# JanWosnitza/FrayTracer

Hardware: AMD Instinct MI355X
Metric: Mrays/s (primary+secondary) at 4096x4096; max per-pixel |delta| vs F# ref (delta is measured against the CPU oracle: F# parity is unpinned, DESIGN.md section 2) (higher is better)
Workload: dtype f32

## Files before the change

fraytracer_amd/csrc/kernels.hip:

```cpp
#include <hip/hip_runtime.h>

#include "../../include/fraytracer_hip.h"
#include "ft_device.h"
#include "ft_kernels.h"
#include "ft_math.h"
#include "ft_libm.h"

#define FT_CONST __attribute__((address_space(4)))
typedef const float FT_CONST* cfp;
template <class T> __device__ __forceinline__ const T FT_CONST* as_const(const T* p) {
    return (const T FT_CONST*)(p);
}

__device__ __forceinline__ f3 ld3(cfp c) { return mk3(c[0], c[1], c[2]); }
__device__ __forceinline__ FtInstr ld_instr(const FtInstr FT_CONST* q) {
    FtInstr r; r.op = q->op; r.dst = q->dst; r.src = q->src; r.type = q->type; r.count = q->count; r.data = q->data;
    r.aux = q->aux; r.flags = q->flags; r.f0 = q->f0; r.f1 = q->f1; r.pad0 = 0; r.pad1 = 0; return r;
}
typedef float v4f __attribute__((ext_vector_type(4)));
typedef uint32_t v4u __attribute__((ext_vector_type(4)));
struct ItemRegs { v4f a; v4u b; };
__device__ __forceinline__ ItemRegs ld_item(const FtItemRec FT_CONST* q) {
    ItemRegs r;
    r.a = *reinterpret_cast<const v4f FT_CONST*>(q);
// ... 990 lines not shown
    float* o = out + 3ull * idx;
    o[0] = c.x; o[1] = c.y; o[2] = c.z;
}

__device__ __forceinline__ f3 ft_background(const FtRenderArgs& a) { return mk3(a.S.bg[0], a.S.bg[1], a.S.bg[2]); }

__device__ __forceinline__ const FtRenderArgs& ft_args_reread() {
    const FtRenderArgs FT_CONST* p = (const FtRenderArgs FT_CONST*)__builtin_amdgcn_kernarg_segment_ptr();
    asm volatile("" : "+s"(p));
    return *(const FtRenderArgs*)p;
}
#define FT_ARGS_AT_USE(on, a) ((on) ? ft_args_reread() : (a))

template <bool EXT>
__device__ __forceinline__ void emit(const FtRenderArgs& a, const LaneState& s, f3 c) {
    write_rgb(a.out, s.outIdx, EXT ? c * s.thr : c);
}

__device__ __forceinline__ uint32_t ft_glass_hash(uint32_t seed, uint32_t bounce) {
    uint32_t h = seed + (bounce + 1u) * 0x27D4EB2Fu;
    h ^= h >> 16; h *= 0x7FEB352Du; h ^= h >> 15; h *= 0x846CA68Bu; h ^= h >> 16;
    return h;
}

__device__ __forceinline__ void write_try_trace_miss(const FtRenderArgs& a, const LaneState& s) {
    float* o = a.out + 10ull * s.outIdx;
    for (uint32_t i = 0; i < 10u; ++i) o[i] = 0.0f;
}
__device__ __forceinline__ void write_ray(float* o, f3 origin, f3 dir, float len, float eps) {
    o[0] = origin.x; o[1] = origin.y; o[2] = origin.z; o[3] = dir.x; o[4] = dir.y; o[5] = dir.z; o[6] = len; o[7] = eps;
}

template <bool VIEWS = false>
__device__ __forceinline__ bool ends_hit_segment(const FtRenderArgs& a, const LaneState& s) {
    if (VIEWS) return a.hits != 0u && (s.job / a.jobsPerPlane) % a.spp == 0u && s.bounce() == 0u;
    return a.hits != 0u && s.job < a.jobsPerPlane && s.bounce() == 0u;
}
template <bool VIEWS = false>
__device__ __forceinline__ uint32_t hit_index(const FtRenderArgs& a, const LaneState& s) {
    if (!VIEWS) return s.outIdx;
    const uint32_t plane = s.job / a.jobsPerPlane;
    return s.outIdx - (plane - plane / a.spp) * a.planePixels;
}
__device__ __forceinline__ void write_hit_record(const FtRenderArgs& a, uint32_t idx, v4f r0, v4f r1, v4f r2, v4f r3, int32_t handle) {
    if (a.hitsOut != nullptr) {
        v4f* o = reinterpret_cast<v4f*>(a.hitsOut + 16ull * idx);
        o[0] = r0; o[1] = r1; o[2] = r2; o[3] = r3;
    }
    if (a.matOut != nullptr) a.matOut[idx] = handle;
}
__device__ __forceinline__ void write_hit_miss(const FtRenderArgs& a, uint32_t idx) {
    const v4f z = {0.0f, 0.0f, 0.0f, 0.0f};
    write_hit_record(a, idx, z, z, z, z, -1);
}

__device__ __forceinline__ bool ft_never_enters(const FtSceneDev& S, const f3 o, const f3 dir, float eps, float len) {
    if (!(S.escR >= 0.0f) || !(len < 1e9f) || !(eps >= 0.0f) || !(eps <= S.escR)) return false;
    const f3 w = o - mk3(S.escC[0], S.escC[1], S.escC[2]);
    const float re = S.escR + eps;
    const float ww = ft_dot(w, w), cc = ww - re * re, tol = 4e-6f * ww, dd = ft_dot(dir, dir);
    if (!(cc > tol) || !(dd < 1e12f)) return false;
    const bool longRay = dd >= 0.25f && ww <= S.escRho2;
    const bool shortRay = len <= 9.9f * S.escR && 2.0f * (ww + dd * (len * len)) <= 6.2f * (S.escR * S.escR);
    if (!longRay && !shortRay) return false;
    const float b = ft_dot(w, dir);
    if (b >= 0.0f) return true;
    return cc * dd - b * b > tol * dd;
}

__device__ __forceinline__ bool ft_cert_segment(const FtSceneDev& S, bool test, const f3 o, const f3 dir, float eps, float len, uint32_t steps,
                                                float& t0, float& t1) {
    const f3 w = o - mk3(S.escC[0], S.escC[1], S.escC[2]);
    const float ww = ft_dot(w, w), dd = ft_dot(dir, dir), b = ft_dot(w, dir);
    bool ok = test && S.certM >= 0.0f && S.escR >= 0.0f && eps >= 0.0f && eps <= S.escR && len > 0.0f && len < 1e9f && dd >= 0.81f && dd <= 1.44f &&
              ww <= S.certRho2 && steps < FT_STEP_CAP - S.certSteps;
    const float R = (S.escR + eps + S.certClip) * 1.001f;
    const float disc = b * b - dd * (ww - R * R);
    ok = ok && disc > 0.0f;
    const float sq = __builtin_amdgcn_sqrtf(ok ? disc : 0.0f), idd = 1.0f / dd;
    t0 = __builtin_fmaxf((-b - sq) * idd, 0.0f); t1 = __builtin_fminf((sq - b) * idd, len * S.certLenF);
    return ok && t1 > t0;
}

template <class P>
__device__ __forceinline__ float ft_seg_dist2(const P prm, const f3 p0, const f3 sv, const float iss) {
    const float vx = prm.x - p0.x, vy = prm.y - p0.y, vz = prm.z - p0.z;
    float t = __builtin_fmaf(vz, sv.z, __builtin_fmaf(vy, sv.y, vx * sv.x)) * iss;
    t = __builtin_amdgcn_fmed3f(t, 0.0f, 1.0f);
    const float ex = __builtin_fmaf(-t, sv.x, vx), ey = __builtin_fmaf(-t, sv.y, vy), ez = __builtin_fmaf(-t, sv.z, vz);
    return __builtin_fmaf(ez, ez, __builtin_fmaf(ey, ey, ex * ex));
}

__device__ __forceinline__ float ft_cert_threshold(float xt) { return __builtin_amdgcn_exp2f(xt) * 0.9999f; }

__device__ __forceinline__ bool ft_miss_certificate(const FtSceneDev& S, const float* __restrict__ ldsC, bool test, const f3 o, const f3 dir, float eps, float len,
                                                    uint32_t steps) {
    const FtInstr FT_CONST* in = as_const(S.instr);
    const float si = in->f0;
    const uint32_t n = in->count;
    const float4* c = reinterpret_cast<const float4*>(ldsC + in->data);
    float t0, t1;
    bool ok = ft_cert_segment(S, test, o, dir, eps, len, steps, t0, t1);
    const float A = si * 1.44269504f;
    const float xt = A * (eps + S.certM);
    ok = ok && xt >= -100.0f;
    if (__ballot(ok) == 0ull) return false;
    const float thr = ft_cert_threshold(xt);
    const f3 p0 = ok ? o + dir * t0 : mk3(0.0f, 0.0f, 0.0f);
    const f3 sv = ok ? dir * (t1 - t0) : mk3(1.0f, 0.0f, 0.0f);
    const float iss = 1.0f / ft_dot(sv, sv);
    float sum = 0.0f;
    uint32_t i = 0;
    auto term = [&](const auto prm) { return __builtin_amdgcn_exp2f((__builtin_amdgcn_sqrtf(ft_seg_dist2(prm, p0, sv, iss)) - prm.w) * A); };
    if (S.certK != 0u) {
        const v4f FT_CONST* cl = reinterpret_cast<const v4f FT_CONST*>(as_const(S.certCl));
        const v4f FT_CONST* kid = cl + 2u * S.certK;
        const float mthr = thr * (0.5f / (float)S.certK);
        float all = 0.0f, rest = 0.0f;
        uint32_t mark = 0u;
        for (uint32_t k = 0; k < S.certK; ++k) {
            const float bnd = term(cl[2u * k]) * (float)__float_as_uint(cl[2u * k + 1u].x);
            all += bnd;
            if (bnd >= mthr) mark |= 1u << k;
            else rest += bnd;
        }
        const bool held = ok && all < thr, open = ok && !held;
        if (__ballot(open) == 0ull) return held;
        float exact = 0.0f;
        for (uint32_t k = 0; k < S.certK; ++k) {
            const bool mine = (mark >> k) & 1u;
            if (__ballot(open && mine) == 0ull) continue;
            const v4f r = cl[2u * k + 1u];
            const uint32_t cnt = __float_as_uint(r.x), first = __float_as_uint(r.y);
            float part = 0.0f;
            for (uint32_t j = 0; j < cnt; ++j) part += term(kid[first + j]);
            exact += mine ? part : 0.0f;
            if (__ballot(open && exact < thr) == 0ull) return held;
        }
        return held || (open && rest + exact < thr);
    }
    for (; i + 8u <= n; i += 8u) {
#pragma unroll
        for (int j = 0; j < 8; ++j) sum += term(c[i + j]);
        if (__ballot(ok && sum < thr) == 0ull) return false;
    }
    for (; i < n; ++i) sum += term(c[i]);
    return ok && sum < thr;
}

__device__ __forceinline__ int ft_axis_lane(unsigned long long mm) {
    return (mm >> 27) != 0ull ? 26 + __ffsll((long long)(mm >> 27)) : __ffsll((long long)mm) - 1;
}

template <bool LEAN = false>
__device__ __forceinline__ bool ft_bundle_certificate(const FtSceneDev& S, const float* __restrict__ ldsC, bool cand, const f3 o, const f3 dir, float eps, float len,
                                                      uint32_t steps, uint32_t minMembers) {
    float t0, t1;
    const bool mem = ft_cert_segment(S, cand, o, dir, eps, len, steps, t0, t1);
    const unsigned long long mm = __ballot(mem);
    if (mm == 0ull || (uint32_t)__popcll(mm) < minMembers) return false;
    const FtInstr FT_CONST* in = as_const(S.instr);
    const float A = in->f0 * 1.44269504f;
    const uint32_t n = in->count;
    const float4* c = reinterpret_cast<const float4*>(ldsC + in->data);
    const int ax = ft_axis_lane(mm);
    const f3 oc = ft_readlane3(o, ax), dc = ft_readlane3(dir, ax);
    const float tc0 = ft_readlane_f(t0, ax), tc1 = ft_readlane_f(t1, ax);
    const f3 g = o - oc, h = dir - dc;
    const float sl = ft_dot(g, dc) * (1.0f / ft_dot(dc, dc));
    const float ex = __builtin_fmaf(-sl, dc.x, g.x), ey = __builtin_fmaf(-sl, dc.y, g.y), ez = __builtin_fmaf(-sl, dc.z, g.z);
    const float al = __builtin_amdgcn_sqrtf(__builtin_fmaf(ez, ez, __builtin_fmaf(ey, ey, ex * ex)));
    const float bl = __builtin_amdgcn_sqrtf(__builtin_fmaf(h.z, h.z, __builtin_fmaf(h.y, h.y, h.x * h.x)));
    const float Wr = ft_wave_max<LEAN>(mem ? __builtin_fmaf(bl, t1, al) : 0.0f);
    const float epsMax = ft_wave_max<LEAN>(mem ? eps : 0.0f);
    const float Rc = (S.escR + epsMax + S.certClip) * 1.001f;
    const float W = Wr * 1.001f + (1e-6f + 4e-6f * Rc);
    const float xt = A * (epsMax + S.certM);
    if (!(W <= S.escR) || !(xt >= -100.0f)) return false;
    const float dLo = ft_wave_max<LEAN>(mem ? __builtin_fmaxf(tc1 - (sl + t0), 0.0f) : 0.0f);
    const float dHi = ft_wave_max<LEAN>(mem ? __builtin_fmaxf((sl + t1) - tc0, 0.0f) : 0.0f);
    const float i0 = (tc1 - dLo) - 4e-6f * Rc, i1 = (tc0 + dHi) + 4e-6f * Rc;
    const f3 p0 = oc + dc * i0, sv = dc * (i1 - i0);
    const float iss = 1.0f / ft_dot(sv, sv);
    const float thr = ft_cert_threshold(xt);
    const uint32_t lane = threadIdx.x & 63u;
    float sum = 0.0f;
    for (uint32_t base = 0; base < n; base += 64u) {
        const uint32_t i = base + lane;
        const float4 prm = c[i < n ? i : n - 1u];
        const float term = __builtin_amdgcn_exp2f((__builtin_amdgcn_sqrtf(ft_seg_dist2(prm, p0, sv, iss)) - (prm.w + W)) * A);
        sum += i < n ? term : 0.0f;
        if (LEAN && __ballot(sum >= thr) != 0ull) return false;
    }
    float total;
    ft_wave_scan_incl(sum, total);
    return mem && total < thr;
}

template <bool LEAN = false>
__device__ __forceinline__ bool ft_occlusion_certificate(const FtRenderArgs& a, const float* __restrict__ ldsC, bool cand, const f3 o, const f3 dir, float eps, float len,
                                                         uint32_t steps) {
    const FtSceneDev& S = a.S;
    const f3 w = o - mk3(S.escC[0], S.escC[1], S.escC[2]);
    const float dd = ft_dot(dir, dir);
    const bool ok = cand && a.occ.b >= 0.0f && S.escR >= 0.0f && eps >= a.occ.epsMin && eps <= S.escR && len > 0.0f && len < 1e9f && dd >= 0.81f && dd <= 1.000001f &&
                    ft_dot(w, w) <= S.certRho2 && steps < FT_STEP_CAP / 2u;
    const unsigned long long mm = __ballot(ok);
    if (mm == 0ull) return false;
    const FtInstr FT_CONST* in = as_const(S.instr);
    const uint32_t n = in->count;
    const float si = in->f0;
    const float4* c = reinterpret_cast<const float4*>(ldsC + in->data);
    const float tEnd = len * a.occ.lenInv;
    const int ax = ft_axis_lane(mm);
    const f3 oc = ft_readlane3(o, ax), dc = ft_readlane3(dir, ax);
    const float tc = ft_readlane_f(tEnd, ax), idc = 1.0f / ft_dot(dc, dc);
    const uint32_t lane = threadIdx.x & 63u;
    auto approach = [](const f3 p, const f3 q, const f3 e, const float ie, const float tMaxi, float& t) {
        const float vx = p.x - q.x, vy = p.y - q.y, vz = p.z - q.z;
        t = __builtin_amdgcn_fmed3f(__builtin_fmaf(vz, e.z, __builtin_fmaf(vy, e.y, vx * e.x)) * ie, 0.0f, tMaxi);
        const float ex = __builtin_fmaf(-t, e.x, vx), ey = __builtin_fmaf(-t, e.y, vy), ez = __builtin_fmaf(-t, e.z, vz);
        return __builtin_amdgcn_sqrtf(__builtin_fmaf(ez, ez, __builtin_fmaf(ey, ey, ex * ex)));
    };
    float best = 0.0f, tAx;
    uint32_t bi = 0u;
    for (uint32_t base = 0; base < n; base += 64u) {
        const uint32_t i = base + lane;
        const float4 prm = c[i < n ? i : n - 1u];
        const float nr = (prm.w + a.occ.near) - approach(mk3(prm.x, prm.y, prm.z), oc, dc, idc, tc, tAx);
        if (i < n && nr > best) { best = nr; bi = i; }
    }
    const float nearest = ft_wave_max<LEAN>(best);
    if (!(nearest > 0.0f)) return false;
    const int src = __ffsll((long long)__ballot(best == nearest)) - 1;
    const float4 sp = c[(uint32_t)__builtin_amdgcn_readlane((int)bi, src)];
    (void)approach(mk3(sp.x, sp.y, sp.z), oc, dc, idc, tc, tAx);
    const f3 y = oc + dc * tAx;
    const float A = si * 1.44269504f;
    float sum = 0.0f;
    for (uint32_t base = 0; base < n; base += 64u) {
        const uint32_t i = base + lane;
        const float4 prm = c[i < n ? i : n - 1u];
        const float dx = prm.x - y.x, dy = prm.y - y.y, dz = prm.z - y.z;
        const float term = __builtin_amdgcn_exp2f((__builtin_amdgcn_sqrtf(__builtin_fmaf(dz, dz, __builtin_fmaf(dy, dy, dx * dx))) - prm.w) * A);
        sum += i < n ? term : 0.0f;
    }
    float total;
    ft_wave_scan_incl(sum, total);
    const float D = __builtin_amdgcn_logf(total) * (-0.693147181f / si);
    const float ie = 1.0f / eps, idd = 1.0f / dd;
    float t;
    bool holds = false;
    {
        const float dist = approach(mk3(sp.x, sp.y, sp.z), o, dir, idd, tEnd, t);
        const float nSteps = __builtin_fmaf(t, ie, 2.0f), hitM = __builtin_fmaf(a.occ.e, nSteps, a.occ.b);
        holds = t <= a.occ.reach && nSteps < 131072.0f && hitM <= a.occ.cap && (dist + hitM) * 1.001f < sp.w;
    }
    {
        const float dist = approach(y, o, dir, idd, tEnd, t);
        const float nSteps = __builtin_fmaf(t, ie, 2.0f), hitM = __builtin_fmaf(a.occ.e, nSteps, a.occ.b);
        holds = holds || (t <= a.occ.reach && nSteps < 131072.0f && hitM <= a.occ.cap && (dist + hitM) * 1.001f < D);
    }
    return ok && holds;
}

__device__ __forceinline__ int first_step_from_cache(LaneState& s) {
    if (s.len <= 0.0f) return 0;
    const float d = *ft_sh(FT_SH_D0);
    if (d != d) { ft_flag(1u); return 2; }
    if (d < s.eps) return 1;
    s.o = s.o + s.dir * d;
    s.len = s.len - d;
    s.steps = 1;
    return 0;
}

struct FtLit { f3 lint, ldir; };
__device__ __forceinline__ FtLit ft_light_at(const uint32_t type, const f3 lv, const f3 lc, const f3 hp) {
    f3 lint = lc, ldir = lv;
    if (type != FT_LIGHT_DIRECTIONAL) { ldir = ft_normalize(lv - hp); lint = lint / ft_length2(lv - hp); }
    return FtLit{lint, ldir};
}

template <bool EXT, int FORM = FT_FORM_FRAME, bool LEAN = false>
__device__ __forceinline__ void settle(const FtRenderArgs& a, LaneState& s) {
    constexpr bool VIEWS = FORM == FT_FORM_VIEWS, SHADE = FORM == FT_FORM_SHADE || FORM == FT_FORM_VIS, VIS = FORM == FT_FORM_VIS;
    const float piInv = 1.0f / 3.14159274101257324f;
    const FtRenderArgs* u = &a;
    for (;;) {
        if (!SHADE && s.phase == PH_MARCH) {
            if (s.len <= 0.0f || ((!EXT || !s.inside()) && ft_never_enters(a.S, s.o, s.dir, s.eps, s.len))) {
                if (LEAN) u = &ft_args_reread();
                if (EXT && u->mode == 2u) write_try_trace_miss(*u, s);
                else {
                    if (EXT && ends_hit_segment<VIEWS>(*u, s)) write_hit_miss(*u, hit_index<VIEWS>(*u, s));
                    if (!EXT || u->hits != 2u) emit<EXT>(*u, s, ft_background(*u));
                }
                s.phase = PH_IDLE;
            }
            return;
        }
        if (EXT && s.phase == PH_AO) {
            if (s.len <= 0.0f) { s.xs += 0x101u; s.phase = PH_AONEXT; continue; }
            return;
        }
        if (EXT && s.phase == PH_AONEXT) {
            if (s.aoIdx() >= a.aoSamples) {
                const float f = (float)s.aoOpen() / (float)a.aoSamples;
                sh_set3(FT_SH_LACC, ft_background(a) * f);
                s.lidx = 0; s.phase = PH_LIGHTS;
                continue;
            }
            const f3 dir = ft_normalize(sh_get3(FT_SH_NRM) + mk3(FT_AO_DIRS[s.aoIdx()][0], FT_AO_DIRS[s.aoIdx()][1], FT_AO_DIRS[s.aoIdx()][2]));
            ft_count(FT_C_EXT);
            if (dir.x != dir.x || dir.y != dir.y || dir.z != dir.z) { s.xs += 0x101u; continue; }
            s.o = sh_get3(FT_SH_HP); s.dir = dir; s.len = a.aoRadius; s.steps = 0;
            s.phase = PH_AO;
            if (a.reuse != 0u) {
                const int r = first_step_from_cache(s);
                if (r == 1) { s.xs += 1u; s.phase = PH_AONEXT; }
                else if (r == 2) s.len = -1.0f;
            }
            continue;
        }
        if (s.phase == PH_SHADOW) {
            if (s.len <= 0.0f || ((!EXT || !s.inside()) && ft_never_enters(a.S, s.o, s.dir, s.eps, s.len))) {
                if (LEAN) u = &ft_args_reread();
                if (VIS) {
                    *ft_vis_word() |= 1u << s.lidx;
                    s.lidx += 1; s.phase = PH_LIGHTS;
                    continue;
                }
                const FtLight L = ld_light(as_const(u->S.lights) + s.lidx);
                const f3 lv = mk3(L.v[0], L.v[1], L.v[2]), hp = sh_get3(FT_SH_HP);
                const FtLit li = ft_light_at(L.type, lv, mk3(L.color[0], L.color[1], L.color[2]), hp);
                sh_set3(FT_SH_LACC, sh_get3(FT_SH_LACC) + li.lint * ft_dot(sh_get3(FT_SH_NRM), li.ldir));
                s.lidx += 1; s.phase = PH_LIGHTS;
                continue;
            }
            return;
        }
        if (s.phase == PH_LIGHTS) {
            if (LEAN) u = &ft_args_reread();
            if (VIS && s.lidx >= u->S.nLights) {
                u->visOut[s.job] = *ft_vis_word();
                s.phase = PH_IDLE;
                return;
            }
            if (VIS && ((u->visSel >> s.lidx) & 1u) == 0u) { s.lidx += 1; continue; }
            if (!VIS && s.lidx >= u->S.nLights) {
                cfp m = SHADE ? as_const(u->hitsIn) + 16ull * s.job + 11u : as_const(u->S.materials) + 3u * s.leaf;
                const f3 color = mk3(m[0], m[1], m[2]);
                emit<EXT>(*u, s, color * (sh_get3(FT_SH_LACC) * piInv));
                s.phase = PH_IDLE;
                return;
            }
            const FtLight L = ld_light(as_const(u->S.lights) + s.lidx);
            const f3 lv = mk3(L.v[0], L.v[1], L.v[2]);
            const f3 hp = sh_get3(FT_SH_HP);
            const f3 ldir = ft_light_at(L.type, lv, mk3(L.color[0], L.color[1], L.color[2]), hp).ldir;
            const float lightCos = ft_dot(sh_get3(FT_SH_NRM), ldir);
            if (lightCos > 0.0f) {
                s.o = hp;
                if (L.type == FT_LIGHT_DIRECTIONAL) {
                    s.dir = lv; s.len = 1000.0f;
                } else {
                    const f3 diff = lv - hp;
                    const float distance2 = ft_length2(diff);
                    s.dir = diff / distance2;
                    s.len = sqrtf(distance2);
                }
                s.steps = 0; ft_count(FT_C_SHADOW);
                s.phase = PH_SHADOW; s.certAt = u->certShadow;
                if (!SHADE && u->reuse != 0u) {
                    const int r = first_step_from_cache(s);
                    if (r == 1) { ft_count(FT_C_HITS); s.lidx += 1; s.phase = PH_LIGHTS; }
                    else if (r == 2) s.len = -1.0f;
                }
                continue;
            }
            s.lidx += 1;
            continue;
        }
        return;
    }
}

struct ViewCam { f3 o, fw, up, rt; float d; uint32_t leaf; };

template <bool EXT, int FORM = FT_FORM_FRAME, bool LEAN = false>
__device__ __forceinline__ void start_job(const FtRenderArgs& a_, LaneState& s, const bool camKnown, float dCam, uint32_t leafCam, const ViewCam& vc) {
    constexpr bool VIEWS = FORM == FT_FORM_VIEWS, SHADE = FORM == FT_FORM_SHADE || FORM == FT_FORM_VIS, VIS = FORM == FT_FORM_VIS;
    const FtRenderArgs& a = FT_ARGS_AT_USE(LEAN, a_);
// ... 109 lines not shown
    s.xs += 0x10000u;
    s.len = a.length; s.steps = 0;
    s.phase = PH_MARCH; s.certAt = a.certPrim;
}

__device__ __forceinline__ void ft_wave_word_add(uint32_t* word, uint32_t v) {
    if ((threadIdx.x & 63u) == 0u) __hip_atomic_fetch_add(word, v, __ATOMIC_RELAXED, __HIP_MEMORY_SCOPE_WORKGROUP);
}

__device__ __forceinline__ unsigned long long wave_sum(uint32_t v) {
    unsigned long long x = v;
    for (int off = 32; off > 0; off >>= 1) x += __shfl_down(x, off, 64);
    return x;
}

__device__ __forceinline__ bool ft_try_due(uint32_t h, uint32_t n, uint32_t r) {
    if (r % FT_HINT_IDLE == 0u) return true;
    if (h != FT_HINT_NONE && (r + 1u == h || r == h)) return true;
    const uint32_t from = n != FT_HINT_NONE ? n : h;
    return from != FT_HINT_NONE && r > from && (r - from) % FT_HINT_AFTER == 0u;
}

template <int VARIANT, bool EXT, int MATH = 0, int K = 0, int FORM = FT_FORM_FRAME>
__device__ __forceinline__ void ft_trace_body(const FtRenderArgs& a) {
    constexpr bool VIEWS = FORM == FT_FORM_VIEWS, SHADE = FORM == FT_FORM_SHADE || FORM == FT_FORM_VIS;
    static_assert(!SHADE || !EXT, "ft_shade_hits and ft_light_visibility have no EXTENSION build");
    constexpr bool LEAN = VARIANT == 1 && !EXT;
    const uint32_t tid = threadIdx.x, lane = tid & 63u;
    unsigned long long* clk0 = reinterpret_cast<unsigned long long*>(ft_lds + 32);
    if (blockIdx.x == 0 && tid == 0) { clk0[0] = clock64(); clk0[1] = wall_clock64(); }
    const FtLdsLayout L = ft_lds_layout(a.S.nSlots, a.S.nStage, MATH != 0, true);
    float* sd = ft_lds + L.slotD + tid;
    uint32_t* sl = reinterpret_cast<uint32_t*>(ft_lds + L.slotL) + tid;
    float* ldsC = ft_lds + L.consts;
    for (uint32_t i = tid; i < a.S.nStage; i += FT_BLOCK) ldsC[i] = a.S.consts[i];
    if (MATH != 0 && tid < FT_LIBM_TAB_DOUBLES) const_cast<ft_u64*>(ft_libm_tab(a.S))[tid] = ft_libm_tab_g[tid];
    if (tid < 32u || (LEAN && (tid - FT_LDS_WAVE_WORD < 4u * (FT_BLOCK / 64) || tid == FT_LDS_REPORT_WORD))) reinterpret_cast<uint32_t*>(ft_lds)[tid] = 0u;
#ifdef FT_UNION_PROFILE
    for (uint32_t k = 0; k < FT_LDS_DBG_ROWS; ++k) reinterpret_cast<uint32_t*>(ft_lds)[FT_LDS_CNT_WORDS + tid + k * FT_BLOCK] = 0u;
#endif
    __syncthreads();
    if (LEAN && blockIdx.x == 0 && tid == 0) reinterpret_cast<uint32_t*>(ft_lds)[FT_LDS_REPORT_WORD] = 1u;

    float* coopRow = ft_lds + ft_lds_layout(a.S.nSlots, a.S.nStage, MATH != 0, true).rows + (uint32_t)__builtin_amdgcn_readfirstlane((int)(tid >> 6)) * FT_CULL_ROW;
    uint32_t cullSkipped = 0, cullTotal = 0;
    uint32_t chunkNext = 0, chunkEnd = 0;
    uint32_t waveEvals = 0;
    constexpr bool ORDER = FORM == FT_FORM_FRAME && !EXT && VARIANT == 1;
    uint32_t* tileSt = reinterpret_cast<uint32_t*>(ft_lds) + FT_LDS_TILE_WORD + (tid >> 6);
    constexpr uint32_t TILE_EVALS = FT_BLOCK / 64;
    if (ORDER && lane == 0) tileSt[0] = 0xffffffffu;
    uint32_t* hintSt = reinterpret_cast<uint32_t*>(ft_lds) + FT_LDS_HINT_WORD + (tid >> 6);
    constexpr uint32_t HINT_NOTE = FT_BLOCK / 64;
    uint32_t coopEvals = 0;
    uint32_t nEvals = 0;
    uint32_t* waveSt = reinterpret_cast<uint32_t*>(ft_lds) + FT_LDS_WAVE_WORD + (tid >> 6);
    enum : uint32_t { ST_EVALS = 0, ST_COOP = FT_BLOCK / 64, ST_CULL_TOTAL = 2 * (FT_BLOCK / 64), ST_CULL_SKIPPED = 3 * (FT_BLOCK / 64) };
    bool exhausted = false;
    LaneState s;
    s.phase = PH_IDLE; s.job = 0; s.steps = 0; s.lidx = 0; s.leaf = 0; s.outIdx = 0; s.certAt = 0xffffffffu;
    s.o = s.dir = mk3(0, 0, 0);
    s.len = 0; s.eps = 0;
    s.xs = 0;
    s.thr = splat3(1.0f); s.seed = 0;
    bool camKnown = false;
    float dCam = 0.0f; uint32_t leafCam = 0u;
    if (!SHADE && a.reuse != 0u && a.mode == 0u) {
        s.phase = PH_CAM;
        if (VIEWS) { const float* c = a.views + 12u * (lane % a.nViews); s.o = mk3(c[0], c[1], c[2]); }
        else s.o = mk3(a.cam[0], a.cam[1], a.cam[2]);
        s.eps = a.eps;
    }
    ViewCam vc{};

    for (;;) {
        for (int round = 0; round < 3; ++round) {
            const unsigned long long idle = __ballot(s.phase == PH_IDLE);
            if (idle == 0ull) break;
            if ((uint32_t)__popcll(idle) < a.refillMin && __ballot(s.phase >= PH_MARCH) != 0ull) break;
            if (chunkNext == chunkEnd) {
                if (exhausted) break;
                const FtRenderArgs& u = FT_ARGS_AT_USE(LEAN, a);
                if (ORDER && u.tileCost != nullptr && lane == 0) {
                    const uint32_t t = tileSt[0];
                    if (t < (u.nJobs >> 6)) {
                        u.tileCost[t] = waveEvals - tileSt[TILE_EVALS];
                        if (u.tileHint != nullptr) u.tileHint[t] = hintSt[HINT_NOTE];
                    }
                    tileSt[0] = 0xffffffffu;
                }
                uint32_t base = 0, take = u.chunk;
                if (lane == 0) {
                    if (u.shrink1 < u.nJobs) {
                        const uint32_t cur = __hip_atomic_load(u.counter, __ATOMIC_RELAXED, __HIP_MEMORY_SCOPE_AGENT);
                        take = cur >= u.shrink2 ? u.chunk / 4u : (cur >= u.shrink1 ? u.chunk / 2u : u.chunk);
                    }
                    base = atomicAdd(u.counter, take);
                }
                base = __builtin_amdgcn_readfirstlane(base);
                const uint32_t took = (uint32_t)__builtin_amdgcn_readfirstlane((int)take);
                if (base >= u.nJobs) { exhausted = true; break; }
                chunkNext = base;
                chunkEnd = (u.nJobs - base < took) ? u.nJobs : base + took;
                if (ORDER && u.tileCost != nullptr) {
                    uint32_t tile = base >> 6;
                    if (u.tileOrder != nullptr) {
                        tile = (uint32_t)__builtin_amdgcn_readfirstlane((int)u.tileOrder[tile]);
                        chunkNext = tile << 6; chunkEnd = chunkNext + 64u;
                    }
                    if (lane == 0) {
                        tileSt[0] = tile; tileSt[TILE_EVALS] = waveEvals;
                        hintSt[0] = u.tryHint != 0u ? (u.tileHint[tile] & 0xffffu) | FT_HINT_USED : 0u;
                        hintSt[HINT_NOTE] = ft_hint_pack(FT_HINT_NONE, FT_HINT_NONE);
                    }
                }
            }
            uint32_t avail = chunkEnd - chunkNext;
            if (VIEWS && a.mode == 0u) {
                const uint32_t jobsPerView = a.jobsPerPlane * (EXT ? a.spp : 1u);
                const uint32_t v = chunkNext / jobsPerView, viewEnd = (v + 1u) * jobsPerView;
                if (viewEnd - chunkNext < avail) avail = viewEnd - chunkNext;
                cfp c = as_const(a.views) + 12u * v;
                vc.o = ld3(c); vc.fw = ld3(c + 3); vc.up = ld3(c + 6); vc.rt = ld3(c + 9);
                vc.d = ft_readlane_f(dCam, (int)v); vc.leaf = (uint32_t)__builtin_amdgcn_readlane((int)leafCam, (int)v);
            }
            const uint32_t nIdle = (uint32_t)__popcll(idle);
            const uint32_t rank = (uint32_t)__popcll(idle & ((1ull << lane) - 1ull));
            if (s.phase == PH_IDLE && rank < avail) { s.job = chunkNext + rank; start_job<EXT, FORM, LEAN>(a, s, camKnown, dCam, leafCam, vc); }
            chunkNext += (nIdle < avail) ? nIdle : avail;
        }
        if (s.phase == PH_IDLE && exhausted && chunkNext == chunkEnd) s.phase = PH_DONE;
        if (__ballot(s.phase != PH_DONE) == 0ull) break;

        if (VARIANT == 1 && FT_WORD_AT_USE(LEAN, a.occPeriod) != 0u && waveEvals % a.occPeriod == 0u) {
            const bool cand = s.phase == PH_SHADOW && s.steps - a.occFrom < a.occPeriod && (!EXT || !s.inside());
            if ((uint32_t)__popcll(__ballot(cand)) >= a.occMin) {
                const bool hit = ft_occlusion_certificate<LEAN>(FT_ARGS_AT_USE(LEAN, a), ldsC + 0, cand, s.o, s.dir, s.eps, s.len, s.steps);
                if (hit) { ft_count(FT_C_HITS); s.lidx += 1; s.phase = PH_LIGHTS; settle<EXT, FORM, LEAN>(a, s); }
                if (__ballot(hit) != 0ull && __ballot(s.phase >= PH_MARCH) == 0ull) continue;
            }
        }

        if (VARIANT == 1 && FT_WORD_AT_USE(LEAN, a.cert) != 0u) {
            bool ends = false;
            const uint32_t hint = ORDER ? (uint32_t)__builtin_amdgcn_readfirstlane((int)hintSt[0]) : 0u;
            const uint32_t noted = ORDER ? (uint32_t)__builtin_amdgcn_readfirstlane((int)hintSt[HINT_NOTE]) : 0u;
            const uint32_t tileRound = ORDER ? waveEvals - (uint32_t)__builtin_amdgcn_readfirstlane((int)tileSt[TILE_EVALS]) : 0u;
            if (FT_WORD_AT_USE(LEAN, a.bundlePeriod) != 0u && ((ORDER && hint != 0u) || waveEvals % a.bundlePeriod == 0u)) {
#pragma unroll 1
                for (uint32_t ph = SHADE ? PH_SHADOW : PH_MARCH; ph <= PH_SHADOW; ph += PH_SHADOW - PH_MARCH) {
                    if (ORDER && hint != 0u && !ft_try_due(ph == PH_MARCH ? ft_hint_primary(hint) : ft_hint_shadow(hint), ph == PH_MARCH ? ft_hint_primary(noted) : ft_hint_shadow(noted), tileRound)) continue;
                    const bool cand = s.phase == ph && (ph == PH_MARCH || s.steps >= a.bundleShadow) && (!EXT || !s.inside());
                    if ((uint32_t)__popcll(__ballot(cand)) < a.bundleMin) continue;
                    const bool held = ft_bundle_certificate<LEAN>(FT_ARGS_AT_USE(LEAN, a).S, ldsC + 0, cand, s.o, s.dir, s.eps, s.len, s.steps, a.bundleMin);
                    if (held) ends = true;
                    if (ORDER && __ballot(held) != 0ull && lane == 0) hintSt[HINT_NOTE] = ft_hint_note(hintSt[HINT_NOTE], ph == PH_MARCH, tileRound);
                }
            }
            const bool due = !ends && (s.phase == PH_MARCH || s.phase == PH_SHADOW) && s.steps >= s.certAt && (!EXT || !s.inside());
            bool tried = false;
            if ((uint32_t)__popcll(__ballot(due)) >= a.certMin) {
                tried = true;
                const FtRenderArgs& u = FT_ARGS_AT_USE(LEAN, a);
                const bool holds = ft_miss_certificate(u.S, ldsC + 0, due, s.o, s.dir, s.eps, s.len, s.steps);
                if (due) {
                    if (holds) ends = true;
                    else s.certAt = u.certRepeat != 0u ? s.steps + u.certRepeat : 0xffffffffu;
                }
            }
            if (ends) { s.len = -1.0f; settle<EXT, FORM, LEAN>(a, s); }
            if ((tried || __ballot(ends) != 0ull) && __ballot(s.phase >= PH_MARCH) == 0ull) continue;
        }

        const bool active = s.phase >= PH_MARCH;
        waveEvals += 1;
        FT_UDBG_T0(tRound);
        auto query_point = [&]() {
            f3 q = s.o;
            if (!SHADE && s.phase >= PH_NX && s.phase <= PH_NC) {
                const f3 base = s.o + s.dir * (-s.eps);
                const float h = s.eps * 0.125f;
                q = base;
                if (s.phase == PH_NX) q.x = base.x + h;
                if (s.phase == PH_NY) q.y = base.y + h;
                if (s.phase == PH_NZ) q.z = base.z + h;
            }
            return q;
        };
        const unsigned long long am = __ballot(active);
        const bool camRound = __ballot(s.phase == PH_CAM) != 0ull;
        if (LEAN) { if (!camRound) ft_wave_word_add(waveSt + ST_EVALS, (uint32_t)__popcll(am)); }
        else if (!camRound) nEvals += (uint32_t)__popcll(am);
        const bool coop = (uint32_t)__popcll(am) <= a.tailK;
        float dCoop = 0.0f; uint32_t leafCoop = 0;
        if (coop && am != 0ull) {
            const f3 qm = query_point();
            if (VARIANT == 1) {
                ft_eval_smooth_spheres_packed<MATH>(a.S, qm, active, am, (uint32_t)__popcll(am), ldsC, coopRow, dCoop, leafCoop);
                if (LEAN) { if (!camRound) ft_wave_word_add(waveSt + ST_COOP, (uint32_t)__popcll(am)); }
                else if (!camRound) coopEvals += (uint32_t)__popcll(am);
            } else {
                unsigned long long m = am;
                while (m != 0ull) {
                    const int L = __ffsll((long long)m) - 1;
                    m &= m - 1ull;
                    const f3 qL = ft_readlane3(qm, L);
                    float dL; uint32_t leafL;
                    if (VARIANT == 3) ft_eval_carved<K, true>(a.S, a.carve, qL, dL, leafL, __builtin_inff());
                    else ft_eval<VARIANT == 2, MATH, true>(a.S, qL, sd, sl, ldsC, dL, leafL);
                    if ((int)lane == L) { dCoop = dL; leafCoop = leafL; }
                    if (!camRound) coopEvals += 1;
                }
            }
        }
        uint32_t cullN = FT_CULL_NONE;
        if (VARIANT != 3 && FT_WORD_AT_USE(LEAN, a.cull) != 0u && !coop && am != 0ull) {
            cullN = ft_cull_children<LEAN>(a.S, query_point(), active, am, ldsC, coopRow);
            if (cullN != FT_CULL_NONE) {
                const uint32_t cnt = (as_const(a.S.instr) + a.S.cullPc)->count;
                const uint32_t looked = cnt < FT_CULL_MAX ? cnt : FT_CULL_MAX;
                const uint32_t total = looked * (uint32_t)__popcll(am) >> 6, skipped = (looked - (cullN & 0xffffu)) * (uint32_t)__popcll(am) >> 6;
                if (LEAN) { ft_wave_word_add(waveSt + ST_CULL_TOTAL, total); ft_wave_word_add(waveSt + ST_CULL_SKIPPED, skipped); }
                else { cullTotal += total; cullSkipped += skipped; }
            }
        }
        if (active) {
            float d; uint32_t leaf;
            FT_UDBG_T0(tEval);
            if (coop) { d = dCoop; leaf = leafCoop; }
            else {
                const f3 q = query_point();
                if (VARIANT == 1) ft_eval_smooth_spheres<MATH, LEAN>(a.S, q, ldsC, d, leaf, coopRow, cullN);
                else if (VARIANT == 3) ft_eval_carved<K>(a.S, a.carve, q, d, leaf, a.lazy == 0u ? __builtin_inff() : s.eps);
                else ft_eval<VARIANT == 2, MATH>(a.S, q, sd, sl, ldsC, d, leaf,
                                                  (EXT && s.inside()) || a.lazy == 0u ? __builtin_inff() : s.eps, coopRow, cullN);
            }
            FT_UDBG_T1(5, tEval); FT_UDBG_WAVE(6);
            if (EXT) d = __uint_as_float(__float_as_uint(d) ^ (s.xs & 0x80000000u));

            const uint32_t ph = SHADE ? (uint32_t)PH_SHADOW : s.phase;
            switch (ph) {
            case PH_MARCH:
            case PH_SHADOW:
            case PH_AO: {
                bool miss = false;
                if (d != d) { ft_flag(1u); miss = true; }
                else if (d < s.eps) {
                    if (ph == PH_MARCH) {
                        ft_count(FT_C_HITP); s.leaf = leaf; s.phase = PH_NX;
                        if (EXT && a.mode == 2u) {
                            float* o = a.out + 10ull * s.outIdx;
                            write_ray(o, s.o, s.dir, s.len, s.eps);
                            o[8] = d; reinterpret_cast<int32_t*>(o)[9] = 1;
                            s.phase = PH_IDLE;
                        }
                    }
                    else if (ph == PH_SHADOW) { ft_count(FT_C_HITS); s.lidx += 1; s.phase = PH_LIGHTS; }
                    else { s.xs += 1u; s.phase = PH_AONEXT; }
                } else {
                    s.o = s.o + s.dir * d;
                    s.len = s.len - d;
                    s.steps += 1;
                    if (s.steps >= FT_STEP_CAP) { ft_flag(4u); miss = true; }
                }
                if (miss) s.len = -1.0f;
                break;
            }
            case PH_CAM:
                if (VIEWS) { dCam = d; leafCam = leaf; }
                else { dCam = ft_readlane_f(d, 0); leafCam = (uint32_t)__builtin_amdgcn_readlane((int)leaf, 0); }
                camKnown = true;
                s.phase = PH_IDLE;
                break;
            case PH_NX: *ft_sh(FT_SH_NRM) = d; s.phase = PH_NY; break;
            case PH_NY: *ft_sh(FT_SH_NRM + 1) = d; s.phase = PH_NZ; break;
            case PH_NZ: *ft_sh(FT_SH_NRM + 2) = d; s.phase = PH_NC; break;
            case PH_NC: {
                *ft_sh(FT_SH_D0) = d;
                const f3 nrm = ft_normalize(sh_get3(FT_SH_NRM) - splat3(d));
                const f3 hp = s.o + s.dir * (-s.eps);
                sh_set3(FT_SH_NRM, nrm);
                sh_set3(FT_SH_HP, hp);
                sh_set3(FT_SH_LACC, ft_background(a));
                s.lidx = 0;
                s.phase = PH_LIGHTS;
                if (EXT && ends_hit_segment<VIEWS>(a, s)) {
                    cfp m = as_const(a.S.materials) + 3u * s.leaf;
                    const float len = s.len - (-s.eps);
                    write_hit_record(a, hit_index<VIEWS>(a, s), v4f{hp.x, hp.y, hp.z, s.dir.x}, v4f{s.dir.y, s.dir.z, len, s.eps},
                                     v4f{nrm.x, nrm.y, nrm.z, m[0]}, v4f{m[1], m[2], __int_as_float(1), 0.0f}, as_const(a.matHandles)[s.leaf]);
                    if (a.hits == 2u) s.phase = PH_IDLE;
                }
                if (EXT && a.aoSamples != 0u) { s.xs &= 0xffff0000u; s.phase = PH_AONEXT; }
                if (EXT && a.maxBounces != 0u) glass_bounce(a, s);
                break;
            }
            default: break;
            }
            settle<EXT, FORM, LEAN>(a, s);
        }
        FT_UDBG_T1(7, tRound);
    }

    const uint32_t* cw = reinterpret_cast<const uint32_t*>(ft_lds) + (tid >> 6);
    if (LEAN) { nEvals = waveSt[ST_EVALS]; coopEvals = waveSt[ST_COOP]; cullTotal = waveSt[ST_CULL_TOTAL]; cullSkipped = waveSt[ST_CULL_SKIPPED]; }
    const unsigned long long e = nEvals, sh = cw[FT_C_SHADOW * 4], hp = cw[FT_C_HITP * 4], hs = cw[FT_C_HITS * 4], pr = cw[FT_C_PRIMARY * 4], ex = cw[FT_C_EXT * 4];
    const unsigned long long fl = cw[FT_C_FLAGS * 4] & 3u, fc = cw[FT_C_FLAGS * 4] & 4u;
    if (lane == 0) {
        const FtRenderArgs& u = FT_ARGS_AT_USE(LEAN, a);
        atomicAdd(&u.stats->sdf_evals, e);
        atomicAdd(&u.stats->rays_shadow, sh);
        atomicAdd(&u.stats->hits_primary, hp);
        atomicAdd(&u.stats->hits_shadow, hs);
        atomicAdd(&u.stats->rays_primary, pr);
        if (ex) atomicAdd(&u.stats->rays_ext, ex);
        atomicAdd(&u.stats->wave_evals, (unsigned long long)waveEvals);
        if (coopEvals) atomicAdd(&u.stats->coop_evals, (unsigned long long)coopEvals);
        if (cullTotal) { atomicAdd(&u.stats->cull_total, (unsigned long long)cullTotal); atomicAdd(&u.stats->cull_skipped, (unsigned long long)cullSkipped); }
        if (fl | fc) atomicOr(&u.stats->flags, fl | fc);
        if (LEAN ? (tid == 0 && reinterpret_cast<const uint32_t*>(ft_lds)[FT_LDS_REPORT_WORD] != 0u) : (blockIdx.x == 0 && tid == 0)) { atomicAdd(&u.stats->clk_shader, clock64() - clk0[0]); atomicAdd(&u.stats->clk_ref, wall_clock64() - clk0[1]); }
    }
#ifdef FT_UNION_PROFILE
    for (uint32_t k = 0; k < 12; ++k) {
        const unsigned long long v = wave_sum(reinterpret_cast<const uint32_t*>(ft_lds)[FT_LDS_CNT_WORDS + tid + k * FT_BLOCK]);
        if (lane == 0 && v) atomicAdd(&ft_union_dbg[k], v);
    }
#endif
}

#ifndef FT_GENERAL_WAVES
#define FT_GENERAL_WAVES 6
#endif
#define FT_OCC(n) __attribute__((amdgpu_waves_per_eu(n, n)))
#ifndef FT_CALLS_WAVES
#define FT_CALLS_WAVES 5
#endif
#ifndef FT_EXT_WAVES
#define FT_EXT_WAVES 5
#endif
#define FT_CALLS_OCC FT_OCC(FT_CALLS_WAVES)
#define FT_EXT_OCC FT_OCC(FT_EXT_WAVES)

#define FT_TRACE_BUILDS(X, ...) \
     \
    X(__VA_ARGS__, , FT_OCC(FT_GENERAL_WAVES), 0, false, 0, 0) \
     \
    X(__VA_ARGS__, _smooth_spheres, , 1, false, 0, 0) \
     \
     \
    X(__VA_ARGS__, _ext, FT_EXT_OCC, 0, true, 0, 0) \
    X(__VA_ARGS__, _smooth_spheres_ext, , 1, true, 0, 0) \
     \
    X(__VA_ARGS__, _calls, FT_CALLS_OCC, 2, false, 0, 0) \
     \
    X(__VA_ARGS__, _calls_ext, FT_OCC(4), 2, true, 0, 0) \
     \
     \
     \
     \
     \
    X(__VA_ARGS__, _carved_spheres, FT_OCC(6), 3, false, 0, FT_PR_SPHERE) \
    X(__VA_ARGS__, _carved_capsules, FT_OCC(6), 3, false, 0, FT_PR_CAPSULE) \
    X(__VA_ARGS__, _carved_tori, FT_OCC(6), 3, false, 0, FT_PR_TORUS) \
    X(__VA_ARGS__, _carved_triangles, FT_OCC(5), 3, false, 0, FT_PR_TRIANGLE) \
    X(__VA_ARGS__, _carved_mixed, FT_OCC(5), 3, false, 0, FT_CARVE_MIXED)       \
     \
     \
    X(__VA_ARGS__, _libm, , 0, false, 1, 0) \
    X(__VA_ARGS__, _smooth_spheres_libm, , 1, false, 1, 0) \
    X(__VA_ARGS__, _ext_libm, , 0, true, 1, 0) \
    X(__VA_ARGS__, _smooth_spheres_ext_libm, , 1, true, 1, 0) \
    X(__VA_ARGS__, _calls_libm, , 2, false, 1, 0) \
    X(__VA_ARGS__, _calls_ext_libm, , 2, true, 1, 0)
#define FT_ROWS_ALL_false(...) __VA_ARGS__
#define FT_ROWS_ALL_true(...) __VA_ARGS__
#define FT_ROWS_NO_EXT_false(...) __VA_ARGS__
#define FT_ROWS_NO_EXT_true(...)
#define FT_TRACE_FORMS(X) \
    FT_TRACE_BUILDS(X, FT_FORM_FRAME, , FT_ROWS_ALL) \
    FT_TRACE_BUILDS(X, FT_FORM_VIEWS, _views, FT_ROWS_ALL) \
    FT_TRACE_BUILDS(X, FT_FORM_SHADE, _shade, FT_ROWS_NO_EXT) \
    FT_TRACE_BUILDS(X, FT_FORM_VIS, _vis, FT_ROWS_NO_EXT)

#define FT_TRACE_KERNEL(FORM, suffix, rows, stem, occ, VARIANT, EXT, MATH, K) \
// ... 724 lines not shown
```

Measured before the change: 1259.

## Split certificate loops into unguarded full-wave chunks and hoist per-round query point

In LEAN mode, the bundle and occlusion certificate loops first run over full 64-element chunks without bounds clamping or select, then fall back to the guarded tail loop. The bundle certificate can also take a uniform eps from the render args in frame mode instead of doing a wave max reduction. The query point is computed once per round into qRound and reused by the coop eval, the cull and the main eval, instead of calling the lambda several times. These remove per-iteration index clamping and redundant reductions and recomputation, at the cost of more code and a risk if eps is not actually uniform.

Measured after the change: 1257. Within noise of the previous version (-0.2%).

```diff
diff --git a/fraytracer_amd/csrc/kernels.hip b/fraytracer_amd/csrc/kernels.hip
--- a/fraytracer_amd/csrc/kernels.hip
+++ b/fraytracer_amd/csrc/kernels.hip
@@ -1166,9 +1166,9 @@
     return (mm >> 27) != 0ull ? 26 + __ffsll((long long)(mm >> 27)) : __ffsll((long long)mm) - 1;
 }
 
-template <bool LEAN = false>
+template <bool LEAN = false, bool ONE_EPS = false>
 __device__ __forceinline__ bool ft_bundle_certificate(const FtSceneDev& S, const float* __restrict__ ldsC, bool cand, const f3 o, const f3 dir, float eps, float len,
-                                                      uint32_t steps, uint32_t minMembers) {
+                                                      uint32_t steps, uint32_t minMembers, const bool oneEps = false, const float epsOne = 0.0f) {
     float t0, t1;
     const bool mem = ft_cert_segment(S, cand, o, dir, eps, len, steps, t0, t1);
     const unsigned long long mm = __ballot(mem);
@@ -1186,7 +1186,7 @@
     const float al = __builtin_amdgcn_sqrtf(__builtin_fmaf(ez, ez, __builtin_fmaf(ey, ey, ex * ex)));
     const float bl = __builtin_amdgcn_sqrtf(__builtin_fmaf(h.z, h.z, __builtin_fmaf(h.y, h.y, h.x * h.x)));
     const float Wr = ft_wave_max<LEAN>(mem ? __builtin_fmaf(bl, t1, al) : 0.0f);
-    const float epsMax = ft_wave_max<LEAN>(mem ? eps : 0.0f);
+    const float epsMax = ONE_EPS && oneEps ? epsOne : ft_wave_max<LEAN>(mem ? eps : 0.0f);
     const float Rc = (S.escR + epsMax + S.certClip) * 1.001f;
     const float W = Wr * 1.001f + (1e-6f + 4e-6f * Rc);
     const float xt = A * (epsMax + S.certM);
@@ -1199,7 +1199,16 @@
     const float thr = ft_cert_threshold(xt);
     const uint32_t lane = threadIdx.x & 63u;
     float sum = 0.0f;
-    for (uint32_t base = 0; base < n; base += 64u) {
+    uint32_t done = 0;
+    if (LEAN) {
+        const float4* cl = c + lane;
+        for (; done + 64u <= n; done += 64u) {
+            const float4 prm = cl[done];
+            sum += __builtin_amdgcn_exp2f((__builtin_amdgcn_sqrtf(ft_seg_dist2(prm, p0, sv, iss)) - (prm.w + W)) * A);
+            if (__ballot(sum >= thr) != 0ull) return false;
+        }
+    }
+    for (uint32_t base = LEAN ? done : 0u; base < n; base += 64u) {
         const uint32_t i = base + lane;
         const float4 prm = c[i < n ? i : n - 1u];
         const float term = __builtin_amdgcn_exp2f((__builtin_amdgcn_sqrtf(ft_seg_dist2(prm, p0, sv, iss)) - (prm.w + W)) * A);
@@ -1238,7 +1247,16 @@
     };
     float best = 0.0f, tAx;
     uint32_t bi = 0u;
-    for (uint32_t base = 0; base < n; base += 64u) {
+    uint32_t doneA = 0, doneB = 0;
+    if (LEAN) {
+        const float4* cl = c + lane;
+        for (; doneA + 64u <= n; doneA += 64u) {
+            const float4 prm = cl[doneA];
+            const float nr = (prm.w + a.occ.near) - approach(mk3(prm.x, prm.y, prm.z), oc, dc, idc, tc, tAx);
+            if (nr > best) { best = nr; bi = doneA + lane; }
+        }
+    }
+    for (uint32_t base = LEAN ? doneA : 0u; base < n; base += 64u) {
         const uint32_t i = base + lane;
         const float4 prm = c[i < n ? i : n - 1u];
         const float nr = (prm.w + a.occ.near) - approach(mk3(prm.x, prm.y, prm.z), oc, dc, idc, tc, tAx);
@@ -1252,7 +1270,15 @@
     const f3 y = oc + dc * tAx;
     const float A = si * 1.44269504f;
     float sum = 0.0f;
-    for (uint32_t base = 0; base < n; base += 64u) {
+    if (LEAN) {
+        const float4* cl = c + lane;
+        for (; doneB + 64u <= n; doneB += 64u) {
+            const float4 prm = cl[doneB];
+            const float dx = prm.x - y.x, dy = prm.y - y.y, dz = prm.z - y.z;
+            sum += __builtin_amdgcn_exp2f((__builtin_amdgcn_sqrtf(__builtin_fmaf(dz, dz, __builtin_fmaf(dy, dy, dx * dx))) - prm.w) * A);
+        }
+    }
+    for (uint32_t base = LEAN ? doneB : 0u; base < n; base += 64u) {
         const uint32_t i = base + lane;
         const float4 prm = c[i < n ? i : n - 1u];
         const float dx = prm.x - y.x, dy = prm.y - y.y, dz = prm.z - y.z;
@@ -1668,7 +1694,9 @@
                     if (ORDER && hint != 0u && !ft_try_due(ph == PH_MARCH ? ft_hint_primary(hint) : ft_hint_shadow(hint), ph == PH_MARCH ? ft_hint_primary(noted) : ft_hint_shadow(noted), tileRound)) continue;
                     const bool cand = s.phase == ph && (ph == PH_MARCH || s.steps >= a.bundleShadow) && (!EXT || !s.inside());
                     if ((uint32_t)__popcll(__ballot(cand)) < a.bundleMin) continue;
-                    const bool held = ft_bundle_certificate<LEAN>(FT_ARGS_AT_USE(LEAN, a).S, ldsC + 0, cand, s.o, s.dir, s.eps, s.len, s.steps, a.bundleMin);
+                    const FtRenderArgs& u = FT_ARGS_AT_USE(LEAN, a);
+                    const bool held = ft_bundle_certificate<LEAN, LEAN && FORM == FT_FORM_FRAME>(u.S, ldsC + 0, cand, s.o, s.dir, s.eps, s.len, s.steps, a.bundleMin,
+                                                                                                  LEAN && u.mode == 0u, u.eps);
                     if (held) ends = true;
                     if (ORDER && __ballot(held) != 0ull && lane == 0) hintSt[HINT_NOTE] = ft_hint_note(hintSt[HINT_NOTE], ph == PH_MARCH, tileRound);
                 }
@@ -1703,6 +1731,18 @@
             }
             return q;
         };
+        f3 qRound = s.o;
+        if (LEAN && !SHADE) {
+            const bool probe = s.phase >= PH_NX && s.phase <= PH_NC;
+            if (__ballot(probe) != 0ull) {
+                const f3 base = s.o + s.dir * (-s.eps);
+                const float h = s.eps * 0.125f;
+                if (probe) qRound = base;
+                if (s.phase == PH_NX) qRound.x = base.x + h;
+                if (s.phase == PH_NY) qRound.y = base.y + h;
+                if (s.phase == PH_NZ) qRound.z = base.z + h;
+            }
+        }
         const unsigned long long am = __ballot(active);
         const bool camRound = __ballot(s.phase == PH_CAM) != 0ull;
         if (LEAN) { if (!camRound) ft_wave_word_add(waveSt + ST_EVALS, (uint32_t)__popcll(am)); }
@@ -1710,7 +1750,7 @@
         const bool coop = (uint32_t)__popcll(am) <= a.tailK;
         float dCoop = 0.0f; uint32_t leafCoop = 0;
         if (coop && am != 0ull) {
-            const f3 qm = query_point();
+            const f3 qm = LEAN ? qRound : query_point();
             if (VARIANT == 1) {
                 ft_eval_smooth_spheres_packed<MATH>(a.S, qm, active, am, (uint32_t)__popcll(am), ldsC, coopRow, dCoop, leafCoop);
                 if (LEAN) { if (!camRound) ft_wave_word_add(waveSt + ST_COOP, (uint32_t)__popcll(am)); }
@@ -1731,7 +1771,7 @@
         }
         uint32_t cullN = FT_CULL_NONE;
         if (VARIANT != 3 && FT_WORD_AT_USE(LEAN, a.cull) != 0u && !coop && am != 0ull) {
-            cullN = ft_cull_children<LEAN>(a.S, query_point(), active, am, ldsC, coopRow);
+            cullN = ft_cull_children<LEAN>(a.S, LEAN ? qRound : query_point(), active, am, ldsC, coopRow);
             if (cullN != FT_CULL_NONE) {
                 const uint32_t cnt = (as_const(a.S.instr) + a.S.cullPc)->count;
                 const uint32_t looked = cnt < FT_CULL_MAX ? cnt : FT_CULL_MAX;
@@ -1745,7 +1785,7 @@
             FT_UDBG_T0(tEval);
             if (coop) { d = dCoop; leaf = leafCoop; }
             else {
-                const f3 q = query_point();
+                const f3 q = LEAN ? qRound : query_point();
                 if (VARIANT == 1) ft_eval_smooth_spheres<MATH, LEAN>(a.S, q, ldsC, d, leaf, coopRow, cullN);
                 else if (VARIANT == 3) ft_eval_carved<K>(a.S, a.carve, q, d, leaf, a.lazy == 0u ? __builtin_inff() : s.eps);
                 else ft_eval<VARIANT == 2, MATH>(a.S, q, sd, sl, ldsC, d, leaf,
```
